# evandez/neuron-descriptions

Measured on AMD Instinct MI355X. Metric: neuron-descriptions/sec (whole node), 4096 neurons x k=15 exemplars, higher is better.
Workload: dtype f32-equivalent: operands split into (hi,lo) f16 pairs (22 significant bits), 3 f16 MFMAs per product, f32 accumulate

## Files before the change

### neuron-descriptions_amd/csrc/api.hip

```cpp
#include "common.h"

#include <cstdarg>
#include <cstdio>
#include <cstring>

namespace milan {

static thread_local char g_err[1024] = "";

void set_error(const char* fmt, ...) {
  va_list ap;
  va_start(ap, fmt);
  vsnprintf(g_err, sizeof(g_err), fmt, ap);
  va_end(ap);
}

int dev_alloc(milan_ctx* c, void** p, size_t bytes) {
  if (bytes == 0) bytes = 16;
  MILAN_CHECK_HIP(hipMalloc(p, (bytes + 255) & ~size_t(255)));
  c->owned.push_back(*p);
  return 0;
}

__global__ void absmax_kernel(const float* __restrict__ w, long n,
// ... 371 lines not shown
  MILAN_REQUIRE(c && seqs && out, MILAN_ERR_ARG,
                "milan_lm_logprobs: null argument");
  set_status_word(c->status);
  Arena a;
  MILAN_TRY(make_arena(workspace, workspace_bytes, &a));
  return decoder_lm_logprobs(c, seqs, rows, L, out, a, (hipStream_t)stream);
}

int milan_conv2d_nhwc(const float* x, int n, int h, int w, int cin,
                      const float* weight_oihw, const float* bias, int cout,
                      int kh, int kw, int stride, int pad, int relu,
                      const float* residual, float* y, int precision,
                      milan_stream stream) {
  MILAN_REQUIRE(x && weight_oihw && y, MILAN_ERR_ARG, "conv2d: null argument");
  set_status_word(nullptr);
  const bool force_strip = precision == 3, tap_major = precision == 4;
  if (force_strip || tap_major) precision = MILAN_PRECISION_SPLIT_F16;
  MILAN_REQUIRE(!force_strip || MILAN_EXPERIMENTS, MILAN_ERR_ARG,
                "conv2d: the LDS-strip 3x3 kernel is only in an experiments build "
                "(make EXPERIMENTS=1)");
  MILAN_REQUIRE(precision == MILAN_PRECISION_F32 || cin % 32 == 0,
                MILAN_ERR_SHAPE, "conv2d: split-f16 needs cin %% 32 == 0");
  MILAN_REQUIRE(cin % 4 == 0 && n > 0 && cout > 0, MILAN_ERR_SHAPE,
                "conv2d: cin must be a multiple of 4");
  hipStream_t s = (hipStream_t)stream;
  const int K = kh * kw * cin, Kp = (K + 31) / 32 * 32;
  float *wp = nullptr, *zero = nullptr, *xs = nullptr, *wsp = nullptr, *ws3 = nullptr, *wst = nullptr;
  MILAN_CHECK_HIP(hipMalloc((void**)&wp, sizeof(float) * (size_t)cout * Kp));
  MILAN_CHECK_HIP(hipMalloc((void**)&zero, 256));
  MILAN_CHECK_HIP(hipMemsetAsync(zero, 0, 256, s));
  int r = pack_conv_plain(weight_oihw, cout, cin, kh, kw, wp, s);
  if (r == 0) {
// ... 11 lines not shown
      hipError_t e1 = hipMalloc((void**)&xs, sizeof(float) * (size_t)rows * cin);
      hipError_t e2 = hipMalloc((void**)&wsp, sizeof(float) * (size_t)cout * Kp);
      if (e1 != hipSuccess || e2 != hipSuccess) {
        set_error("conv2d: out of memory");
        r = (int)hipErrorOutOfMemory;
      } else {
        r = launch_f32_to_split(x, cin, xs, cin, rows, cin, 1.f, s);
        if (r == 0)
          r = split_weight_into(wp, cout, Kp, wsp, &g.acc_scale,
                                reinterpret_cast<unsigned int*>(zero) + 32, s);
        g.A = xs; g.W = wsp; g.a_split = 1;
        if (r == 0 && !tap_major && kh * kw > 1 && kh * kw <= 32 && K == Kp) {
          if (hipMalloc((void**)&wst, sizeof(float) * (size_t)cout * Kp) == hipSuccess) {
            r = make_slice_major(wsp, cout, kh * kw, cin, 4, 2, wst, s);
            g.Wt = wst;
          }
        }
        if (MILAN_EXPERIMENTS && r == 0 && kh == 3 && kw == 3 && stride == 1 &&
            pad == 1 && K == Kp) {
          if (hipMalloc((void**)&ws3, sizeof(float) * (size_t)cout * Kp) == hipSuccess) {
            r = make_chunk_major(wsp, cout, cin, ws3, s);
            g.W3 = ws3;
            if (force_strip) g.tile_hint = 8;
          }
        }
      }
    }
    if (r == 0) r = launch_gemm(g, s);
  }
  hipError_t e = hipStreamSynchronize(s);
// ... 163 lines not shown
```

### neuron-descriptions_amd/csrc/common.h

```cpp
#pragma once
#include <hip/hip_runtime.h>
#include <stdint.h>
#include <stddef.h>
#include <string>
#include <vector>
#include <map>

#include "../../include/milan_hip.h"

#ifndef MILAN_EXPERIMENTS
#define MILAN_EXPERIMENTS 0
#endif

namespace milan {

void set_error(const char* fmt, ...);
#define MILAN_CHECK_HIP(expr)                                              \
  do {                                                                     \
    hipError_t _e = (expr);                                                \
    if (_e != hipSuccess) {                                                \
      milan::set_error("%s:%d: %s -> %s", __FILE__, __LINE__, #expr,       \
                       hipGetErrorString(_e));                             \
      return (int)_e;                                                      \
    }                                                                      \
// ... 10 lines not shown
    int _r = (expr);                                                       \
    if (_r != 0) return _r;                                                \
  } while (0)

enum Epilogue : int {
  EPI_BIAS = 0,
  EPI_BIAS_RELU = 1,
  EPI_BIAS_RES_RELU = 2,
  EPI_BIAS_TANH = 3,
  EPI_BIAS_SIGMUL = 4,
  EPI_BIAS_ADD = 5,
  EPI_LSTM = 6,
  EPI_LSE = 7,
};

struct GemmArgs {
  const float* A;
  const float* W;
  const float* bias;
  const float* aux;
  float* C;
  int M, N, K, Kp;
  int ldc, ldaux;
  int H, Wd, Cin, Ho, Wo, KH, KW, stride, pad;
  long a_pix_stride;
  long a_img_stride;
  int epilogue;
  const float* zero;
  int flop_k;
  int a_split;
// ... 10 lines not shown
  int tile_hint;
  int stagger;
  long long* prof;
  int chunk_major;
  float* C2;
  float* Cs;
  unsigned* status;
  int f16;
  const float* Wt;
  int tap_inner;
  const long long* lse_tgt;
  long lse_tgt_stride;
  float* lse_x;
  const int* m_live;
  int m_live_mul;
};

enum OutMode : int { OUT_SCALAR = 0, OUT_VEC4 = 1, OUT_SPLIT8 = 2, OUT_F16 = 3 };

int launch_gemm(const GemmArgs& g, hipStream_t s);
void set_status_word(unsigned* word);
unsigned* status_word();
void profile_tag_kernel(int family);
int launch_zero_fill(void* p, size_t bytes, hipStream_t s);
int launch_f32_to_split(const float* src, long ld_src, float* dst, long ld_dst,
                        long rows, int K, float scale, hipStream_t s);
int gemm_profile_enable(int enable);
int ensure_lds_attr(const void* kern, int bytes);
int device_cus8(int* out);
void* gemm_profile_begin(double flops, double bytes, hipStream_t s);
void gemm_profile_end(void* rec, hipStream_t s);
// ... 350 lines not shown
```

### neuron-descriptions_amd/csrc/gemm.hip

```cpp
#include "common.h"

#include <map>
#include <mutex>
#include <utility>

#include <cstdio>
#include <cstdlib>
#include <type_traits>
#include <utility>
#include <vector>

#ifndef MILAN_ABLATE_BUILD
#define MILAN_ABLATE_BUILD 0
#endif
#ifndef MILAN_EXPERIMENTS
#define MILAN_EXPERIMENTS 0
#endif

namespace milan {

typedef float f32x16 __attribute__((ext_vector_type(16)));
typedef float f32x4 __attribute__((ext_vector_type(4)));
typedef _Float16 f16x8 __attribute__((ext_vector_type(8)));

// ... 47 lines not shown
               "s_nop 1\n\tv_max_f32_dpp %0, %0, %0 quad_perm:[2,3,0,1] row_mask:0xf bank_mask:0xf\n\t"
               "s_nop 1\n\tv_max_f32_dpp %0, %0, %0 row_half_mirror row_mask:0xf bank_mask:0xf\n\t"
               "s_nop 1\n\tv_max_f32_dpp %0, %0, %0 row_mirror row_mask:0xf bank_mask:0xf"
               : "+v"(x));
  return x;
}
__device__ __forceinline__ float row16_sum(float x) {
  asm volatile("s_nop 1\n\tv_add_f32_dpp %0, %0, %0 quad_perm:[1,0,3,2] row_mask:0xf bank_mask:0xf\n\t"
               "s_nop 1\n\tv_add_f32_dpp %0, %0, %0 quad_perm:[2,3,0,1] row_mask:0xf bank_mask:0xf\n\t"
               "s_nop 1\n\tv_add_f32_dpp %0, %0, %0 row_half_mirror row_mask:0xf bank_mask:0xf\n\t"
               "s_nop 1\n\tv_add_f32_dpp %0, %0, %0 row_mirror row_mask:0xf bank_mask:0xf"
               : "+v"(x));
  return x;
}

template <int TM, int TN, bool SWZ64 = false>
__device__ __forceinline__ void run_epilogue(const GemmArgs& g,
                                             f32x16 (&acc)[TM][TN], float* smem,
                                             int wave, int lane, int row0,
                                             int col0) {
  static_assert(TN == 2, "epilogues assume 64-column wave tiles");
  constexpr int SROW = SWZ64 ? 64 : 68;
  auto sw = [](int row, int col) { return SWZ64 ? (col ^ ((row & 1) << 2)) : col; };
  float* stage_out = smem + wave * (32 * SROW);
  auto to_stage = [&](int i) {
#pragma unroll
    for (int j = 0; j < TN; ++j)
#pragma unroll
      for (int r = 0; r < 16; ++r) {
        const int row = (r & 3) + 8 * (r >> 2) + 4 * (lane >> 5);
        stage_out[row * SROW + sw(row, j * 32 + (lane & 31))] = acc[i][j][r];
      }
  };

  auto epilogue_vec4 = [&](auto epi_tag) {
    constexpr int EPI = decltype(epi_tag)::value;
    const int col4 = (lane & 15) * 4;
    const int n = col0 + col4;
    const bool n_ok = n < g.N;
    f32x4 bias4 = {0.f, 0.f, 0.f, 0.f};
    if (g.bias && n_ok) bias4 = *reinterpret_cast<const f32x4*>(g.bias + n);
    constexpr bool AUX = (EPI == EPI_BIAS_RES_RELU || EPI == EPI_BIAS_ADD ||
                          EPI == EPI_BIAS_SIGMUL);
    f32x4 res[AUX ? 2 : 1][8];
    auto load_res = [&](int i, f32x4 (&r)[8]) {
#pragma unroll
      for (int it = 0; it < 8; ++it) {
        const int m = row0 + i * 32 + it * 4 + (lane >> 4);
        r[it] = (m < g.M && n_ok)
                    ? *reinterpret_cast<const f32x4*>(g.aux + (long)m * g.ldaux + n)
                    : f32x4{0.f, 0.f, 0.f, 0.f};
      }
    };
    if constexpr (AUX) load_res(0, res[0]);
#pragma unroll
    for (int i = 0; i < TM; ++i) {
      if constexpr (AUX) {
        if (i + 1 < TM) load_res(i + 1, res[(i + 1) & 1]);
      }
      to_stage(i);
#pragma unroll
      for (int it = 0; it < 8; ++it) {
        const int row = it * 4 + (lane >> 4);
        const int m = row0 + i * 32 + row;
        f32x4 v = *reinterpret_cast<const f32x4*>(stage_out + row * SROW + sw(row, col4));
        if (m < g.M && n_ok) {
          v += bias4;
          if constexpr (AUX) {
            const f32x4 a = res[i & 1][it];
            if constexpr (EPI == EPI_BIAS_SIGMUL) {
#pragma unroll
              for (int e = 0; e < 4; ++e)
                v[e] = (1.f / (1.f + expf(-v[e]))) * a[e];
            } else {
              v += a;
            }
          }
          if constexpr (EPI == EPI_BIAS_RELU || EPI == EPI_BIAS_RES_RELU) {
#pragma unroll
// ... 8 lines not shown
      }
    }
  };

  auto epilogue_lse = [&]() {
    const int col4 = (lane & 15) * 4;
    const int n = col0 + col4;
    const bool n_ok = n < g.N;
    f32x4 bias4 = {0.f, 0.f, 0.f, 0.f};
    if (g.bias && n_ok) bias4 = *reinterpret_cast<const f32x4*>(g.bias + n);
    const int cb = col0 >> 6;
    int tg[2][8];
    auto load_tgt = [&](int i, int (&t)[8]) {
#pragma unroll
      for (int it = 0; it < 8; ++it) {
        const int m = row0 + i * 32 + it * 4 + (lane >> 4);
        t[it] = m < g.M ? (int)g.lse_tgt[(long)m * g.lse_tgt_stride] : -1;
      }
    };
    load_tgt(0, tg[0]);
#pragma unroll
    for (int i = 0; i < TM; ++i) {
      if (i + 1 < TM) load_tgt(i + 1, tg[(i + 1) & 1]);
      to_stage(i);
#pragma unroll
      for (int it = 0; it < 8; ++it) {
        const int row = it * 4 + (lane >> 4);
        const int m = row0 + i * 32 + row;
        f32x4 v = *reinterpret_cast<const f32x4*>(stage_out + row * SROW + sw(row, col4));
        v += bias4;
        const bool ok = m < g.M && n_ok;
        float mx = ok ? fmaxf(fmaxf(v[0], v[1]), fmaxf(v[2], v[3])) : -INFINITY;
        mx = row16_max(mx);
        float e = ok ? (__expf(v[0] - mx) + __expf(v[1] - mx)) + (__expf(v[2] - mx) + __expf(v[3] - mx)) : 0.f;
        e = row16_sum(e);
        if (m < g.M && col0 < g.N) {
          if ((lane & 15) == 0) {
            float* d = g.C + (long)m * g.ldc + 2 * cb;
            d[0] = mx;
            d[1] = e;
          }
          const int tgt = tg[i & 1][it];
          if (n_ok && tgt >= n && tgt < n + 4) {
// ... 12 lines not shown
    const bool n_ok = n < g.N;
    float bias8[8] = {0.f, 0.f, 0.f, 0.f, 0.f, 0.f, 0.f, 0.f};
    if (g.bias && n_ok) {
      const f32x4 b0 = *reinterpret_cast<const f32x4*>(g.bias + n);
      const f32x4 b1 = *reinterpret_cast<const f32x4*>(g.bias + n + 4);
#pragma unroll
      for (int e = 0; e < 4; ++e) { bias8[e] = b0[e]; bias8[4 + e] = b1[e]; }
    }
    constexpr bool SIG = EPI == EPI_BIAS_SIGMUL;
    constexpr bool RES = (EPI == EPI_BIAS_RES_RELU || EPI == EPI_BIAS_ADD || SIG);
    float sat = 0.f;
    f32x4 res[RES ? 2 : 1][4][2];
    auto load_res = [&](int i, f32x4 (&r)[4][2]) {
#pragma unroll
      for (int it = 0; it < 4; ++it) {
        const int m = row0 + i * 32 + it * 8 + (lane >> 3);
        if (m < g.M && n_ok) {
          const float* ap = g.aux + (long)m * g.ldaux + n;
          r[it][0] = *reinterpret_cast<const f32x4*>(ap);
          r[it][1] = *reinterpret_cast<const f32x4*>(ap + 4);
        } else {
          r[it][0] = f32x4{0.f, 0.f, 0.f, 0.f};
          r[it][1] = r[it][0];
        }
      }
    };
    if constexpr (RES) load_res(0, res[0]);
#pragma unroll
    for (int i = 0; i < TM; ++i) {
      if constexpr (RES) {
        if (i + 1 < TM) load_res(i + 1, res[(i + 1) & 1]);
      }
      to_stage(i);
#pragma unroll
      for (int it = 0; it < 4; ++it) {
        const int row = it * 8 + (lane >> 3);
        const int m = row0 + i * 32 + row;
        const f32x4 v0 =
            *reinterpret_cast<const f32x4*>(stage_out + row * SROW + sw(row, col8));
        const f32x4 v1 =
            *reinterpret_cast<const f32x4*>(stage_out + row * SROW + sw(row, col8 + 4));
        if (m < g.M && n_ok) {
          float v[8];
#pragma unroll
          for (int e = 0; e < 4; ++e) {
            v[e] = v0[e] + bias8[e];
            v[4 + e] = v1[e] + bias8[4 + e];
          }
          if constexpr (SIG) {
            const f32x4 a0 = res[i & 1][it][0], a1 = res[i & 1][it][1];
#pragma unroll
            for (int e = 0; e < 4; ++e) {
// ... 27 lines not shown
    const int n = col0 + col8;
    const bool n_ok = n < g.N;
    float bias8[8] = {0.f, 0.f, 0.f, 0.f, 0.f, 0.f, 0.f, 0.f};
    if (g.bias && n_ok) {
      const f32x4 b0 = *reinterpret_cast<const f32x4*>(g.bias + n);
      const f32x4 b1 = *reinterpret_cast<const f32x4*>(g.bias + n + 4);
#pragma unroll
      for (int e = 0; e < 4; ++e) { bias8[e] = b0[e]; bias8[4 + e] = b1[e]; }
    }
    constexpr bool RES = EPI == EPI_BIAS_RES_RELU;
    float sat = 0.f;
    f32x4 res[RES ? 2 : 1][4];
    auto load_res = [&](int i, f32x4 (&r)[4]) {
#pragma unroll
      for (int it = 0; it < 4; ++it) {
        const int m = row0 + i * 32 + it * 8 + (lane >> 3);
        r[it] = (m < g.M && n_ok)
                    ? *reinterpret_cast<const f32x4*>(reinterpret_cast<const char*>(g.aux) +
                                                      ((long)m * g.ldaux * 4 + n * 2))
                    : f32x4{0.f, 0.f, 0.f, 0.f};
      }
    };
    if constexpr (RES) load_res(0, res[0]);
#pragma unroll
    for (int i = 0; i < TM; ++i) {
      if constexpr (RES) {
        if (i + 1 < TM) load_res(i + 1, res[(i + 1) & 1]);
      }
      to_stage(i);
#pragma unroll
      for (int it = 0; it < 4; ++it) {
        const int row = it * 8 + (lane >> 3);
        const int m = row0 + i * 32 + row;
        const f32x4 v0 = *reinterpret_cast<const f32x4*>(stage_out + row * SROW + sw(row, col8));
        const f32x4 v1 = *reinterpret_cast<const f32x4*>(stage_out + row * SROW + sw(row, col8 + 4));
        if (m < g.M && n_ok) {
          float v[8];
#pragma unroll
          for (int e = 0; e < 4; ++e) {
            v[e] = v0[e] + bias8[e];
            v[4 + e] = v1[e] + bias8[4 + e];
          }
          if constexpr (RES) {
            const f16x8v a = __builtin_bit_cast(f16x8v, res[i & 1][it]);
#pragma unroll
            for (int e = 0; e < 8; ++e) v[e] += (float)a[e];
          }
          float x[8];
// ... 17 lines not shown

  auto epilogue_lstm = [&]() {
    const int q4 = (lane & 3) * 4;
    const int u = (col0 >> 2) + q4;
    const bool n_ok = col0 < g.N;
    f32x4 bias4[4];
#pragma unroll
    for (int gate = 0; gate < 4; ++gate)
      bias4[gate] = (g.bias && n_ok)
                        ? *reinterpret_cast<const f32x4*>(g.bias + col0 + gate * 16 + q4)
                        : f32x4{0.f, 0.f, 0.f, 0.f};
    f32x4 cin[2][2];
    auto load_c = [&](int i, f32x4 (&c)[2]) {
#pragma unroll
      for (int it = 0; it < 2; ++it) {
        const int m = row0 + i * 32 + it * 16 + (lane >> 2);
        c[it] = (m < g.M && n_ok)
                    ? *reinterpret_cast<const f32x4*>(g.aux + (long)m * g.ldaux + u)
                    : f32x4{0.f, 0.f, 0.f, 0.f};
      }
    };
    load_c(0, cin[0]);
#pragma unroll
    for (int i = 0; i < TM; ++i) {
      if (i + 1 < TM) load_c(i + 1, cin[(i + 1) & 1]);
      to_stage(i);
#pragma unroll
      for (int it = 0; it < 2; ++it) {
        const int row = it * 16 + (lane >> 2);
        const int m = row0 + i * 32 + row;
        f32x4 p[4];
#pragma unroll
        for (int gate = 0; gate < 4; ++gate)
          p[gate] = *reinterpret_cast<const f32x4*>(stage_out + row * SROW +
                                                    sw(row, gate * 16 + q4)) + bias4[gate];
        if (m < g.M && n_ok) {
          f32x4 h4, c4;
#pragma unroll
          for (int e = 0; e < 4; ++e) {
            float hh, cc;
            lstm_cell(p[0][e], p[1][e], p[2][e], p[3][e], cin[i & 1][it][e], &hh, &cc);
            h4[e] = hh; c4[e] = cc;
          }
          *reinterpret_cast<f32x4*>(g.C + (long)m * g.ldc + u) = h4;
          *reinterpret_cast<f32x4*>(g.C2 + (long)m * g.ldc + u) = c4;
// ... 14 lines not shown
          }
        }
      }
    }
  };

  auto epilogue_scalar = [&](auto epi_tag) {
    constexpr int EPI = decltype(epi_tag)::value;
#pragma unroll
    for (int j = 0; j < TN; ++j) {
      const int n = col0 + j * 32 + (lane & 31);
      if (n >= g.N) continue;
      const float bias = g.bias ? g.bias[n] : 0.f;
#pragma unroll
      for (int i = 0; i < TM; ++i) {
        const int mbase = row0 + i * 32 + 4 * (lane >> 5);
#pragma unroll
        for (int r = 0; r < 16; ++r) {
          const int m = mbase + (r & 3) + 8 * (r >> 2);
          if (m >= g.M) continue;
          float v = acc[i][j][r] + bias;
          if constexpr (EPI == EPI_BIAS_RELU) v = fmaxf(v, 0.f);
          if constexpr (EPI == EPI_BIAS_RES_RELU)
            v = fmaxf(v + g.aux[(long)m * g.ldaux + n], 0.f);
          if constexpr (EPI == EPI_BIAS_ADD) v = v + g.aux[(long)m * g.ldaux + n];
          if constexpr (EPI == EPI_BIAS_TANH) v = tanhf(v);
          if constexpr (EPI == EPI_BIAS_SIGMUL)
            v = (1.f / (1.f + expf(-v))) * g.aux[(long)m * g.ldaux + n];
          g.C[(long)m * g.ldc + n] = v;
        }
      }
    }
  };

// ... 988 lines not shown
  __builtin_amdgcn_s_barrier();
  const GemmArgs ge = reload_gemm_args();
#pragma unroll
  for (int i = 0; i < TM; ++i)
#pragma unroll
    for (int j = 0; j < TN; ++j) acc[i][j] = acc[i][j] * ge.acc_scale;
  run_epilogue<TM, TN>(ge, acc, smem, wave, lane, tile_m * BM + wm * 128, tile_n * BN + wn * 64);
}

struct PpLoader {
  __amdgpu_buffer_rsrc_t srd_a, srd_a2, srd_w, cur_srd;
  unsigned row_off[4], row_off2[4], voff[4], vb[4];
  int hw0[4];
  unsigned mask[4];
  int ia, iw, is_kh, is_kw, is_cin0, seg_soff, cin_limit;
};

template <int BNW, bool F16 = false, bool TAPI = false>
__device__ __forceinline__ void split16_pp32_tile(int tile_m, int tile_n, int tid, bool prefetched,
                                                  bool has_next, int ntile_m, int ntile_n) {
  const GemmArgs g = reload_gemm_args();
  constexpr int BM = 256, BN = 256, BKP = 32, TM = BNW == 256 ? 4 : 2, TN = 2;
  static_assert(BNW == 256 || BNW == 128, "ping-pong tile: 256 or 128 columns");
  constexpr int SLOTF = BM * BKP;
  constexpr unsigned OOB = 0x80000000u;
  extern __shared__ __attribute__((aligned(16))) float smem[];
  auto a_slot = [&](int sl) { return smem + (sl < 2 ? sl : 3) * SLOTF; };
  auto w_slot = [&](int sl) { return smem + (sl == 0 ? 2 : 4) * SLOTF; };
  const int lane = tid & 63;
  const int wave = __builtin_amdgcn_readfirstlane(tid >> 6);
  const int wm = BNW == 256 ? wave >> 2 : wave >> 1, wn = BNW == 256 ? wave & 3 : wave & 1;
  const int group = wave >> 2;
  const int HoWo = g.Ho * g.Wo;
  const int np = g.Kp / BKP;
  const int k1_pairs = g.A2 ? g.K1 / BKP : 0x7fffffff;

  auto set_tap = [&](PpLoader& L) {
    if constexpr (TAPI) {
      const int t = L.is_kh * g.KW + L.is_kw;
#pragma unroll
      for (int it = 0; it < 4; ++it) L.voff[it] = (L.mask[it] >> t) & 1u ? L.row_off[it] : OOB;
      L.seg_soff = (int)((((long)L.is_kh * g.Wd + L.is_kw) * g.a_pix_stride) * 4);
      return;
    }
#pragma unroll
    for (int it = 0; it < 4; ++it) {
      const int hi = (L.hw0[it] >> 16) + L.is_kh, wi = (int)(short)(L.hw0[it] & 0xffff) + L.is_kw;
      const bool inb = (unsigned)hi < (unsigned)g.H && (unsigned)wi < (unsigned)g.Wd;
      L.voff[it] = inb ? L.row_off[it] : OOB;
    }
    L.seg_soff = (int)((((long)L.is_kh * g.Wd + L.is_kw) * g.a_pix_stride) * 4);
  };
  auto setup = [&](PpLoader& L, int tm, int tn) {
    const int prow = lane >> 3, pos = lane & 7;
    const int m0 = tm * BM;
    const int img0 = m0 / HoWo;
    const int rem0 = m0 - img0 * HoWo;
    const long bias = ((long)g.pad * g.Wd + g.pad) * g.a_pix_stride;
    L.srd_a = __builtin_amdgcn_make_buffer_rsrc(
        const_cast<float*>(g.A + (long)img0 * g.a_img_stride - bias), 0, 0x7fffffff, 0x00020000);
    L.srd_a2 = __builtin_amdgcn_make_buffer_rsrc(
        const_cast<float*>(g.A2 ? g.A2 + (long)img0 * g.a2_img_stride : g.A), 0, 0x7fffffff,
        0x00020000);
    L.srd_w = __builtin_amdgcn_make_buffer_rsrc(const_cast<float*>(g.W + (long)tn * BNW * g.Kp), 0,
                                                0x7fffffff, 0x00020000);
    const float r_howo = 1.0f / (float)HoWo, r_wo = 1.0f / (float)g.Wo;
#pragma unroll
    for (int it = 0; it < 4; ++it) {
      const int row = it * 64 + wave * 8 + prow;
      const int q = pos ^ ((row >> 1) & 7);
      const bool ok = m0 + row < g.M;
      const int x = rem0 + (ok ? row : 0);
      int dimg = (int)((float)x * r_howo);
      dimg -= (dimg * HoWo > x);
      dimg += ((dimg + 1) * HoWo <= x);
      const int rem = x - dimg * HoWo;
      int ho = (int)((float)rem * r_wo);
      ho -= (ho * g.Wo > rem);
      ho += ((ho + 1) * g.Wo <= rem);
      const int wo = rem - ho * g.Wo;
      const int hi0 = ho * g.stride - g.pad, wi0 = wo * g.stride - g.pad;
      L.hw0[it] = (hi0 << 16) | (wi0 & 0xffff);
      if constexpr (TAPI) {
        unsigned m = 0;
        for (int kh = 0, t = 0; kh < g.KH; ++kh)
          for (int kw = 0; kw < g.KW; ++kw, ++t)
            m |= (unsigned)((unsigned)(hi0 + kh) < (unsigned)g.H &&
                            (unsigned)(wi0 + kw) < (unsigned)g.Wd) << t;
        L.mask[it] = m;
      }
      L.row_off[it] = ok ? (unsigned)(((long)dimg * g.a_img_stride +
                                       ((long)hi0 * g.Wd + wi0) * g.a_pix_stride + bias + q * 4) * 4)
                         : OOB;
      L.row_off2[it] = (ok && g.A2)
                           ? (unsigned)(((long)dimg * g.a2_img_stride +
                                         ((long)(ho * g.stride2) * g.W2d + wo * g.stride2) *
                                             g.a2_pix_stride + q * 4) * 4)
                           : OOB;
      L.vb[it] = (row < BNW && tn * BNW + row < g.N) ? (unsigned)(((long)row * g.Kp + q * 4) * 4) : OOB;
    }
    L.ia = L.iw = L.is_kh = L.is_kw = L.is_cin0 = 0;
    L.cin_limit = g.Cin;
    L.cur_srd = L.srd_a;
    set_tap(L);
  };
  auto issue_a = [&](PpLoader& L, auto slot_tag, bool really) {
    constexpr int SLOT = decltype(slot_tag)::value;
    if (really) {
      int woff = wave * (8 * BKP);
      asm volatile("" : "+s"(woff));
      float* dst = a_slot(SLOT) + woff;
      const int soff = L.seg_soff + L.is_cin0 * 4;
#pragma unroll
      for (int it = 0; it < 4; ++it)
        __builtin_amdgcn_raw_ptr_buffer_load_lds(L.cur_srd, (LDS_AS void*)(dst + it * (64 * BKP)), 16,
                                                 L.voff[it], soff, 0, 0);
    }
    if constexpr (TAPI) {
      if (L.ia + 1 < np) {
        ++L.ia;
        if (++L.is_kw == g.KW) {
          L.is_kw = 0;
          if (++L.is_kh == g.KH) { L.is_kh = 0; L.is_cin0 += BKP; }
        }
        set_tap(L);
      }
      return;
    }
    if (L.ia + 1 < np) {
      ++L.ia;
      L.is_cin0 += BKP;
      if (L.ia == k1_pairs) {
        L.cur_srd = L.srd_a2;
#pragma unroll
        for (int it = 0; it < 4; ++it) L.voff[it] = L.row_off2[it];
        L.seg_soff = 0;
        L.is_cin0 = 0;
        L.cin_limit = 0x7fffffff;
      } else if (L.is_cin0 >= L.cin_limit) {
        L.is_cin0 = 0;
        if (++L.is_kw == g.KW) { L.is_kw = 0; ++L.is_kh; }
        set_tap(L);
      }
    }
  };
  auto issue_w = [&](PpLoader& L, auto slot_tag, bool really) {
    constexpr int SLOT = decltype(slot_tag)::value;
    if (really) {
      int woff = wave * (8 * BKP);
      asm volatile("" : "+s"(woff));
      float* dst = w_slot(SLOT) + woff;
      const int soff = L.iw * (BKP * 4);
#pragma unroll
      for (int it = 0; it < (BNW == 256 ? 4 : 2); ++it)
        __builtin_amdgcn_raw_ptr_buffer_load_lds(L.srd_w, (LDS_AS void*)(dst + it * (64 * BKP)), 16,
                                                 L.vb[it], soff, 0, 0);
    }
    if (L.iw + 1 < np) ++L.iw;
  };
  using I0 = std::integral_constant<int, 0>;
  using I1 = std::integral_constant<int, 1>;

  PpLoader L;
  setup(L, tile_m, tile_n);

  const int frow = lane & 31, fhalf = lane >> 5;
  const int fsw = (frow >> 1) & 7;
  const float* a_p[2][2];
  const float* a_q[2][2];
  const float* b_p[2][2];
  const float* b_q[2][2];
#pragma unroll
  for (int sl = 0; sl < 2; ++sl)
// ... 154 lines not shown
  }
  asm volatile("s_waitcnt vmcnt(0)" ::: "memory");
  __builtin_amdgcn_s_barrier();
  if (has_next) {
    PpLoader N;
    setup(N, ntile_m, ntile_n);
    issue_a(N, I0{}, true);
    issue_w(N, I0{}, true);
    issue_a(N, I1{}, true);
  }
  const GemmArgs ge = reload_gemm_args();
#pragma unroll
  for (int i = 0; i < TM; ++i)
#pragma unroll
    for (int j = 0; j < TN; ++j) acc[i][j] = acc[i][j] * ge.acc_scale;
  run_epilogue<TM, TN, true>(ge, acc, a_slot(2), wave, lane, tile_m * BM + wm * (TM * 32),
                             tile_n * BNW + wn * 64);
}

template <int BNW>
__global__ __launch_bounds__(512, 2) void igemm_split16_pp32n_kernel(GemmArgs g, int tiles_m,
                                                                     int tiles_n) {
  tiles_m = live_tiles_m(g, tiles_m, 256);
  const int T = tiles_m * tiles_n;
  int q = blockIdx.x;
  if (q >= T) return;
  bool prefetched = false;
  for (;;) {
    const int tile = xcd_tile(q, T);
    const int tile_m = tile / tiles_n, tile_n = tile - tile_m * tiles_n;
    const bool has_next = q + (int)gridDim.x < T;
    int ntile_m = tile_m, ntile_n = tile_n;
// ... 18 lines not shown
  tiles_m = live_tiles_m(g, tiles_m, 256);
  const int T = tiles_m * tiles_n;
  const int q = blockIdx.x;
  if (q >= T) return;
  const int tile = xcd_tile(q, T);
  const int tile_m = tile / tiles_n, tile_n = tile - tile_m * tiles_n;
  int tid = threadIdx.x;
  asm volatile("" : "+v"(tid));
  split16_pp32_tile<256>(tile_m, tile_n, tid, false, false, tile_m, tile_n);
}

template <int BNW>
__global__ __launch_bounds__(512, 2) void igemm_split16_pp32t_kernel(GemmArgs g, int tiles_m,
                                                                     int tiles_n) {
  tiles_m = live_tiles_m(g, tiles_m, 256);
  const int T = tiles_m * tiles_n;
  const int q = blockIdx.x;
  if (q >= T) return;
  const int tile = xcd_tile(q, T);
  const int tile_m = tile / tiles_n, tile_n = tile - tile_m * tiles_n;
  int tid = threadIdx.x;
  asm volatile("" : "+v"(tid));
  split16_pp32_tile<BNW, false, true>(tile_m, tile_n, tid, false, false, tile_m, tile_n);
}

template <int BNW, bool TAPI>
__global__ __launch_bounds__(512, 2) void igemm_f16_pp32_kernel(GemmArgs g, int tiles_m, int tiles_n) {
  tiles_m = live_tiles_m(g, tiles_m, 256);
  const int T = tiles_m * tiles_n;
  const int q = blockIdx.x;
  if (q >= T) return;
  const int tile = xcd_tile(q, T);
  const int tile_m = tile / tiles_n, tile_n = tile - tile_m * tiles_n;
  int tid = threadIdx.x;
  asm volatile("" : "+v"(tid));
  split16_pp32_tile<BNW, true, TAPI>(tile_m, tile_n, tid, false, false, tile_m, tile_n);
}

__global__ __launch_bounds__(512, 2) void igemm_split16_pp_kernel(GemmArgs g, int tiles_m,
                                                                  int tiles_n) {
  tiles_m = live_tiles_m(g, tiles_m, 256);
  const int T = tiles_m * tiles_n;
  for (int q = blockIdx.x; q < T; q += gridDim.x) {
    const int tile = xcd_tile(q, T);
    const int tile_m = tile / tiles_n;
    int tid = threadIdx.x;
    asm volatile("" : "+v"(tid));
    split16_pp_tile(tile_m, tile - tile_m * tiles_n, tid);
    __builtin_amdgcn_s_barrier();
  }
}
// ... 465 lines not shown
  auto kern = igemm_split16_tm2_kernel<BM, BN, STAGES>;
  MILAN_TRY(ensure_lds_attr(reinterpret_cast<const void*>(kern), (int)lds));
  hipLaunchKernelGGL(kern, dim3(tiles_m * tiles_n), dim3(NT), lds, s, g, tiles_m,
                     tiles_n);
  MILAN_CHECK_HIP(hipGetLastError());
  return 0;
}

static bool tap_inner_wanted(const GemmArgs& g) {
  static int on = -1;
  if (on < 0) { const char* e = getenv("MILAN_TAP_INNER"); on = e ? atoi(e) : 1; }
  return on && g.Wt && !g.A2 && g.KH * g.KW > 1 && g.KH * g.KW <= 32 && g.K == g.Kp &&
         g.Cin % 32 == 0;
}

template <int BNW>
static int launch_split16_pp32(const GemmArgs& g, hipStream_t s) {
  const int tiles_m = (g.M + 255) / 256, tiles_n = (g.N + BNW - 1) / BNW;
  const size_t lds = size_t(5) * 256 * 32 * sizeof(float);
  if (tap_inner_wanted(g)) {
    GemmArgs t = g;
    t.W = g.Wt;
    t.tap_inner = 1;
    profile_tag_kernel(BNW == 256 ? MILAN_KERNEL_PP32T_256 : MILAN_KERNEL_PP32_128);
    auto kern = igemm_split16_pp32t_kernel<BNW>;
    MILAN_TRY(ensure_lds_attr(reinterpret_cast<const void*>(kern), (int)lds));
    hipLaunchKernelGGL(kern, dim3(tiles_m * tiles_n), dim3(512), lds, s, t, tiles_m, tiles_n);
    MILAN_CHECK_HIP(hipGetLastError());
    return 0;
  }
  int ncus = 0;
  MILAN_TRY(device_cus8(&ncus));
  int grid = tiles_m * tiles_n;
  static int persist = -1;
  if (persist < 0) { const char* e = getenv("MILAN_PP_PERSIST"); persist = e ? atoi(e) : 0; }
  const bool walk = persist && (persist != 2 || g.K <= 512) && grid > ncus;
  profile_tag_kernel(BNW == 256 ? MILAN_KERNEL_PP32_256 : MILAN_KERNEL_PP32_128);
  if (BNW == 256 && !walk) {
    auto kern = igemm_split16_pp32_kernel;
    MILAN_TRY(ensure_lds_attr(reinterpret_cast<const void*>(kern), (int)lds));
    hipLaunchKernelGGL(kern, dim3(grid), dim3(512), lds, s, g, tiles_m, tiles_n);
  } else {
// ... 3 lines not shown
    hipLaunchKernelGGL(kern, dim3(grid), dim3(512), lds, s, g, tiles_m, tiles_n);
  }
  MILAN_CHECK_HIP(hipGetLastError());
  return 0;
}

template <int BNW>
static int launch_f16_pp32(const GemmArgs& g, hipStream_t s) {
  const int tiles_m = (g.M + 255) / 256, tiles_n = (g.N + BNW - 1) / BNW;
  const size_t lds = size_t(5) * 256 * 32 * sizeof(float);
  profile_tag_kernel(MILAN_KERNEL_F16);
  if (tap_inner_wanted(g)) {
    GemmArgs t = g;
    t.W = g.Wt;
    t.tap_inner = 1;
    auto kern = igemm_f16_pp32_kernel<BNW, true>;
    MILAN_TRY(ensure_lds_attr(reinterpret_cast<const void*>(kern), (int)lds));
    hipLaunchKernelGGL(kern, dim3(tiles_m * tiles_n), dim3(512), lds, s, t, tiles_m, tiles_n);
    MILAN_CHECK_HIP(hipGetLastError());
    return 0;
  }
  auto kern = igemm_f16_pp32_kernel<BNW, false>;
  MILAN_TRY(ensure_lds_attr(reinterpret_cast<const void*>(kern), (int)lds));
  hipLaunchKernelGGL(kern, dim3(tiles_m * tiles_n), dim3(512), lds, s, g, tiles_m, tiles_n);
  MILAN_CHECK_HIP(hipGetLastError());
  return 0;
}

static int launch_split16_pp(const GemmArgs& g, hipStream_t s) {
  const int tiles_m = (g.M + 255) / 256, tiles_n = (g.N + 255) / 256;
  const size_t lds = size_t(4) * (256 + 256) * 16 * sizeof(float);
  static_assert(size_t(4) * 512 * 16 * sizeof(float) >= size_t(8) * 32 * 68 * sizeof(float),
                "the epilogue stages through the ring");
// ... 273 lines not shown
```

### neuron-descriptions_amd/milan_amd/hip.py

```python
import ctypes
import os
import pathlib
import weakref
from typing import Dict, Optional, Sequence, Tuple

import torch

LIB_PATH = pathlib.Path(os.environ.get('MILAN_LIB') or
                       pathlib.Path(__file__).resolve().parent / 'lib' / 'libmilan_hip.so')
EXP_LIB_PATH = pathlib.Path(__file__).resolve().parent / 'lib' / 'libmilan_hip_exp.so'

GREEDY, FORCED, BEAM, RERANK = 0, 1, 2, 3
PRECISION_F32, PRECISION_SPLIT_F16, PRECISION_F16 = 0, 1, 2
PRECISIONS = {'f32': PRECISION_F32, 'split_f16': PRECISION_SPLIT_F16, 'f16': PRECISION_F16}
FUSE_CHAIN, FUSE_CHAIN_WIDE, FUSE_STEM, FUSE_CONV3, FUSE_SKIP_EMPTY, FUSE_BNECK, FUSE_SPARSE_TAIL = 1, 2, 4, 8, 16, 32, 64
SKETCH_COMPACT, SKETCH_INSERT, SKETCH_MOVE, SKETCH_HALVE = 0, 1, 2, 3
STATUS_SATURATED, STATUS_NONFINITE_INPUT = 1, 2
KERNEL_FAMILIES = ('other', 'pp32_256', 'pp32_128', 'split_other', 'f32', 'chain',
                   'chain_wide', 'stem', 'conv3', 'f16', 'pp32t_256', 'bneck')


class SketchOp(ctypes.Structure):
    _fields_ = [('kind', ctypes.c_int32), ('src', ctypes.c_int32),
                ('dst', ctypes.c_int32), ('offset', ctypes.c_int32),
                ('extremes', ctypes.c_int32), ('reserved', ctypes.c_int32),
                ('n', ctypes.c_int64), ('position', ctypes.c_int64),
                ('capacity', ctypes.c_int64)]


DRAW_BIT = ctypes.CFUNCTYPE(ctypes.c_int, ctypes.c_void_p)
_CONV_PRECISIONS = dict(f32=0, split_f16=1, split_f16_strip=3, split_f16_tap_major=4)
DTYPE_U8, DTYPE_F32 = 0, 1

ERR_ARG, ERR_SHAPE, ERR_STATE, ERR_WORKSPACE, ERR_NO_LM = -1, -2, -3, -4, -5


class HipUnavailableError(RuntimeError):
    """libmilan_hip.so or a HIP device is missing."""


class Dims(ctypes.Structure):
    _fields_ = [
        ('trunk_width', ctypes.c_int32),
        ('trunk_blocks', ctypes.c_int32 * 4),
        ('feature_size', ctypes.c_int32),
        ('hidden_size', ctypes.c_int32),
# ... 1451 lines not shown
```

Measured before the change: 1313.

## Skip padded taps in tap-inner conv GEMM by grouping output pixels into border classes

Output pixels of the tap-inner implicit-GEMM conv are partitioned into up to nine classes by which kernel taps fall inside the image (interior vs. border rows/columns). Each class gets its own block range and iterates only over its valid taps via a bitmask, so the zero-padding taps at borders are no longer loaded or multiplied. The epilogue now scatters rows through a per-wave LDS row table because a tile no longer covers contiguous output rows. This adds grid bookkeeping, an env toggle, and an extra tile-rounding loss per class, in exchange for skipping the wasted padding work.

```diff
diff --git a/neuron-descriptions_amd/csrc/api.hip b/neuron-descriptions_amd/csrc/api.hip
--- a/neuron-descriptions_amd/csrc/api.hip
+++ b/neuron-descriptions_amd/csrc/api.hip
@@ -409,8 +409,8 @@
                       milan_stream stream) {
   MILAN_REQUIRE(x && weight_oihw && y, MILAN_ERR_ARG, "conv2d: null argument");
   set_status_word(nullptr);
-  const bool force_strip = precision == 3, tap_major = precision == 4;
-  if (force_strip || tap_major) precision = MILAN_PRECISION_SPLIT_F16;
+  const bool force_strip = precision == 3, tap_major = precision == 4, tap_linear = precision == 5;
+  if (force_strip || tap_major || tap_linear) precision = MILAN_PRECISION_SPLIT_F16;
   MILAN_REQUIRE(!force_strip || MILAN_EXPERIMENTS, MILAN_ERR_ARG,
                 "conv2d: the LDS-strip 3x3 kernel is only in an experiments build "
                 "(make EXPERIMENTS=1)");
@@ -452,6 +452,7 @@
           if (hipMalloc((void**)&wst, sizeof(float) * (size_t)cout * Kp) == hipSuccess) {
             r = make_slice_major(wsp, cout, kh * kw, cin, 4, 2, wst, s);
             g.Wt = wst;
+            if (tap_linear) g.tap_ncls = -1;
           }
         }
         if (MILAN_EXPERIMENTS && r == 0 && kh == 3 && kw == 3 && stride == 1 &&
diff --git a/neuron-descriptions_amd/csrc/common.h b/neuron-descriptions_amd/csrc/common.h
--- a/neuron-descriptions_amd/csrc/common.h
+++ b/neuron-descriptions_amd/csrc/common.h
@@ -48,6 +48,7 @@
   EPI_LSE = 7,
 };
 
+constexpr int MILAN_TAP_CLASSES = 9;
 struct GemmArgs {
   const float* A;
   const float* W;
@@ -88,7 +89,10 @@
   float* lse_x;
   const int* m_live;
   int m_live_mul;
-};
+  int tap_ncls;
+  int tap_cls[MILAN_TAP_CLASSES][5];
+};
+static_assert(sizeof(GemmArgs) % 4 == 0, "GemmArgs is reloaded word by word");
 
 enum OutMode : int { OUT_SCALAR = 0, OUT_VEC4 = 1, OUT_SPLIT8 = 2, OUT_F16 = 3 };
 
diff --git a/neuron-descriptions_amd/csrc/gemm.hip b/neuron-descriptions_amd/csrc/gemm.hip
--- a/neuron-descriptions_amd/csrc/gemm.hip
+++ b/neuron-descriptions_amd/csrc/gemm.hip
@@ -6,6 +6,7 @@
 
 #include <cstdio>
 #include <cstdlib>
+#include <cstring>
 #include <type_traits>
 #include <utility>
 #include <vector>
@@ -85,12 +86,16 @@
   return x;
 }
 
-template <int TM, int TN, bool SWZ64 = false>
+template <int TM, int TN, bool SWZ64 = false, bool ROWTAB = false>
 __device__ __forceinline__ void run_epilogue(const GemmArgs& g,
                                              f32x16 (&acc)[TM][TN], float* smem,
                                              int wave, int lane, int row0,
-                                             int col0) {
+                                             int col0, const int* rowtab = nullptr) {
   static_assert(TN == 2, "epilogues assume 64-column wave tiles");
+  auto out_row = [&](int r) {
+    if constexpr (ROWTAB) return rowtab[r];
+    else return row0 + r;
+  };
   constexpr int SROW = SWZ64 ? 64 : 68;
   auto sw = [](int row, int col) { return SWZ64 ? (col ^ ((row & 1) << 2)) : col; };
   float* stage_out = smem + wave * (32 * SROW);
@@ -117,7 +122,7 @@
     auto load_res = [&](int i, f32x4 (&r)[8]) {
 #pragma unroll
       for (int it = 0; it < 8; ++it) {
-        const int m = row0 + i * 32 + it * 4 + (lane >> 4);
+        const int m = out_row(i * 32 + it * 4 + (lane >> 4));
         r[it] = (m < g.M && n_ok)
                     ? *reinterpret_cast<const f32x4*>(g.aux + (long)m * g.ldaux + n)
                     : f32x4{0.f, 0.f, 0.f, 0.f};
@@ -133,7 +138,7 @@
 #pragma unroll
       for (int it = 0; it < 8; ++it) {
         const int row = it * 4 + (lane >> 4);
-        const int m = row0 + i * 32 + row;
+        const int m = out_row(i * 32 + row);
         f32x4 v = *reinterpret_cast<const f32x4*>(stage_out + row * SROW + sw(row, col4));
         if (m < g.M && n_ok) {
           v += bias4;
@@ -172,7 +177,7 @@
     auto load_tgt = [&](int i, int (&t)[8]) {
 #pragma unroll
       for (int it = 0; it < 8; ++it) {
-        const int m = row0 + i * 32 + it * 4 + (lane >> 4);
+        const int m = out_row(i * 32 + it * 4 + (lane >> 4));
         t[it] = m < g.M ? (int)g.lse_tgt[(long)m * g.lse_tgt_stride] : -1;
       }
     };
@@ -184,7 +189,7 @@
 #pragma unroll
       for (int it = 0; it < 8; ++it) {
         const int row = it * 4 + (lane >> 4);
-        const int m = row0 + i * 32 + row;
+        const int m = out_row(i * 32 + row);
         f32x4 v = *reinterpret_cast<const f32x4*>(stage_out + row * SROW + sw(row, col4));
         v += bias4;
         const bool ok = m < g.M && n_ok;
@@ -227,7 +232,7 @@
     auto load_res = [&](int i, f32x4 (&r)[4][2]) {
 #pragma unroll
       for (int it = 0; it < 4; ++it) {
-        const int m = row0 + i * 32 + it * 8 + (lane >> 3);
+        const int m = out_row(i * 32 + it * 8 + (lane >> 3));
         if (m < g.M && n_ok) {
           const float* ap = g.aux + (long)m * g.ldaux + n;
           r[it][0] = *reinterpret_cast<const f32x4*>(ap);
@@ -248,7 +253,7 @@
 #pragma unroll
       for (int it = 0; it < 4; ++it) {
         const int row = it * 8 + (lane >> 3);
-        const int m = row0 + i * 32 + row;
+        const int m = out_row(i * 32 + row);
         const f32x4 v0 =
             *reinterpret_cast<const f32x4*>(stage_out + row * SROW + sw(row, col8));
         const f32x4 v1 =
@@ -306,7 +311,7 @@
     auto load_res = [&](int i, f32x4 (&r)[4]) {
 #pragma unroll
       for (int it = 0; it < 4; ++it) {
-        const int m = row0 + i * 32 + it * 8 + (lane >> 3);
+        const int m = out_row(i * 32 + it * 8 + (lane >> 3));
         r[it] = (m < g.M && n_ok)
                     ? *reinterpret_cast<const f32x4*>(reinterpret_cast<const char*>(g.aux) +
                                                       ((long)m * g.ldaux * 4 + n * 2))
@@ -323,7 +328,7 @@
 #pragma unroll
       for (int it = 0; it < 4; ++it) {
         const int row = it * 8 + (lane >> 3);
-        const int m = row0 + i * 32 + row;
+        const int m = out_row(i * 32 + row);
         const f32x4 v0 = *reinterpret_cast<const f32x4*>(stage_out + row * SROW + sw(row, col8));
         const f32x4 v1 = *reinterpret_cast<const f32x4*>(stage_out + row * SROW + sw(row, col8 + 4));
         if (m < g.M && n_ok) {
@@ -371,7 +376,7 @@
     auto load_c = [&](int i, f32x4 (&c)[2]) {
 #pragma unroll
       for (int it = 0; it < 2; ++it) {
-        const int m = row0 + i * 32 + it * 16 + (lane >> 2);
+        const int m = out_row(i * 32 + it * 16 + (lane >> 2));
         c[it] = (m < g.M && n_ok)
                     ? *reinterpret_cast<const f32x4*>(g.aux + (long)m * g.ldaux + u)
                     : f32x4{0.f, 0.f, 0.f, 0.f};
@@ -385,7 +390,7 @@
 #pragma unroll
       for (int it = 0; it < 2; ++it) {
         const int row = it * 16 + (lane >> 2);
-        const int m = row0 + i * 32 + row;
+        const int m = out_row(i * 32 + row);
         f32x4 p[4];
 #pragma unroll
         for (int gate = 0; gate < 4; ++gate)
@@ -430,10 +435,9 @@
       const float bias = g.bias ? g.bias[n] : 0.f;
 #pragma unroll
       for (int i = 0; i < TM; ++i) {
-        const int mbase = row0 + i * 32 + 4 * (lane >> 5);
 #pragma unroll
         for (int r = 0; r < 16; ++r) {
-          const int m = mbase + (r & 3) + 8 * (r >> 2);
+          const int m = out_row(i * 32 + 4 * (lane >> 5) + (r & 3) + 8 * (r >> 2));
           if (m >= g.M) continue;
           float v = acc[i][j][r] + bias;
           if constexpr (EPI == EPI_BIAS_RELU) v = fmaxf(v, 0.f);
@@ -1452,11 +1456,56 @@
   int hw0[4];
   unsigned mask[4];
   int ia, iw, is_kh, is_kw, is_cin0, seg_soff, cin_limit;
+  unsigned a_bits, w_bits;
+  int w_slice;
 };
+
+struct TapTile {
+  int y0, ny, x0, nx;
+  unsigned mask;
+  int cnt, j, tile_n;
+};
+
+__device__ __forceinline__ bool tap_tile(const GemmArgs& g, int tiles_m, int tiles_n, TapTile* t) {
+  const int b = blockIdx.x;
+  if (g.tap_ncls == 0) {
+    const int T = tiles_m * tiles_n;
+    if (b >= T) return false;
+    const int tile = xcd_tile(b, T);
+    t->j = tile / tiles_n;
+    t->tile_n = tile - t->j * tiles_n;
+    t->y0 = 0; t->ny = g.Ho; t->x0 = 0; t->nx = g.Wo;
+    t->mask = 0xffffffffu >> (32 - g.KH * g.KW);
+    t->cnt = g.M;
+    return true;
+  }
+  typedef const int __attribute__((address_space(4)))* KArgWords;
+  const KArgWords cw = (KArgWords)__builtin_amdgcn_kernarg_segment_ptr() + offsetof(GemmArgs, tap_cls) / 4;
+  const int imgs = g.M / (g.Ho * g.Wo);
+  int first = 0, cls = -1, cfirst = 0, ctiles = 0;
+#pragma unroll
+  for (int c = 0; c < MILAN_TAP_CLASSES; ++c) {
+    const int T = c < g.tap_ncls ? ((imgs * cw[c * 5 + 1] * cw[c * 5 + 3] + 255) >> 8) * tiles_n : 0;
+    const int B = (T + 7) & ~7;
+    if (cls < 0 && b < first + B) { cls = c; cfirst = first; ctiles = T; }
+    first += B;
+  }
+  if (cls < 0) return false;
+  const int bl = b - cfirst;
+  if ((bl >> 3) >= (ctiles >> 3) + ((bl & 7) < (ctiles & 7))) return false;
+  const int tile = xcd_tile(bl, ctiles);
+  t->j = tile / tiles_n;
+  t->tile_n = tile - t->j * tiles_n;
+  t->y0 = cw[cls * 5]; t->ny = cw[cls * 5 + 1]; t->x0 = cw[cls * 5 + 2]; t->nx = cw[cls * 5 + 3];
+  t->mask = (unsigned)cw[cls * 5 + 4];
+  t->cnt = imgs * t->ny * t->nx;
+  return true;
+}
 
 template <int BNW, bool F16 = false, bool TAPI = false>
 __device__ __forceinline__ void split16_pp32_tile(int tile_m, int tile_n, int tid, bool prefetched,
-                                                  bool has_next, int ntile_m, int ntile_n) {
+                                                  bool has_next, int ntile_m, int ntile_n,
+                                                  TapTile tt = TapTile{}) {
   const GemmArgs g = reload_gemm_args();
   constexpr int BM = 256, BN = 256, BKP = 32, TM = BNW == 256 ? 4 : 2, TN = 2;
   static_assert(BNW == 256 || BNW == 128, "ping-pong tile: 256 or 128 columns");
@@ -1470,15 +1519,18 @@
   const int wm = BNW == 256 ? wave >> 2 : wave >> 1, wn = BNW == 256 ? wave & 3 : wave & 1;
   const int group = wave >> 2;
   const int HoWo = g.Ho * g.Wo;
-  const int np = g.Kp / BKP;
+  const int np = TAPI ? (g.Cin / BKP) * __builtin_popcount(tt.mask) : g.Kp / BKP;
   const int k1_pairs = g.A2 ? g.K1 / BKP : 0x7fffffff;
+  const int KHKW = g.KH * g.KW;
+  const int r_kw = 65536 / g.KW + 1;
 
   auto set_tap = [&](PpLoader& L) {
     if constexpr (TAPI) {
-      const int t = L.is_kh * g.KW + L.is_kw;
+      const int t = __builtin_ctz(L.a_bits);
+      const int kh = (t * r_kw) >> 16, kw = t - kh * g.KW;
 #pragma unroll
       for (int it = 0; it < 4; ++it) L.voff[it] = (L.mask[it] >> t) & 1u ? L.row_off[it] : OOB;
-      L.seg_soff = (int)((((long)L.is_kh * g.Wd + L.is_kw) * g.a_pix_stride) * 4);
+      L.seg_soff = (int)((((long)kh * g.Wd + kw) * g.a_pix_stride) * 4);
       return;
     }
 #pragma unroll
@@ -1489,11 +1541,29 @@
     }
     L.seg_soff = (int)((((long)L.is_kh * g.Wd + L.is_kw) * g.a_pix_stride) * 4);
   };
+  const int pix_img = TAPI ? tt.ny * tt.nx : HoWo, pix_row = TAPI ? tt.nx : g.Wo;
+  const int rows_all = TAPI ? tt.cnt : g.M;
+  const float r_howo = 1.0f / (float)pix_img, r_wo = 1.0f / (float)pix_row;
+  auto row_pixel = [&](int m0, int rem0, int row, int* dimg_out, int* ho_out, int* wo_out) {
+    const bool ok = m0 + row < rows_all;
+    const int x = rem0 + (ok ? row : 0);
+    int dimg = (int)((float)x * r_howo);
+    dimg -= (dimg * pix_img > x);
+    dimg += ((dimg + 1) * pix_img <= x);
+    const int rem = x - dimg * pix_img;
+    int ho = (int)((float)rem * r_wo);
+    ho -= (ho * pix_row > rem);
+    ho += ((ho + 1) * pix_row <= rem);
+    *dimg_out = dimg;
+    *wo_out = rem - ho * pix_row + (TAPI ? tt.x0 : 0);
+    *ho_out = ho + (TAPI ? tt.y0 : 0);
+    return ok;
+  };
   auto setup = [&](PpLoader& L, int tm, int tn) {
     const int prow = lane >> 3, pos = lane & 7;
     const int m0 = tm * BM;
-    const int img0 = m0 / HoWo;
-    const int rem0 = m0 - img0 * HoWo;
+    const int img0 = m0 / pix_img;
+    const int rem0 = m0 - img0 * pix_img;
     const long bias = ((long)g.pad * g.Wd + g.pad) * g.a_pix_stride;
     L.srd_a = __builtin_amdgcn_make_buffer_rsrc(
         const_cast<float*>(g.A + (long)img0 * g.a_img_stride - bias), 0, 0x7fffffff, 0x00020000);
@@ -1502,21 +1572,12 @@
         0x00020000);
     L.srd_w = __builtin_amdgcn_make_buffer_rsrc(const_cast<float*>(g.W + (long)tn * BNW * g.Kp), 0,
                                                 0x7fffffff, 0x00020000);
-    const float r_howo = 1.0f / (float)HoWo, r_wo = 1.0f / (float)g.Wo;
 #pragma unroll
     for (int it = 0; it < 4; ++it) {
       const int row = it * 64 + wave * 8 + prow;
       const int q = pos ^ ((row >> 1) & 7);
-      const bool ok = m0 + row < g.M;
-      const int x = rem0 + (ok ? row : 0);
-      int dimg = (int)((float)x * r_howo);
-      dimg -= (dimg * HoWo > x);
-      dimg += ((dimg + 1) * HoWo <= x);
-      const int rem = x - dimg * HoWo;
-      int ho = (int)((float)rem * r_wo);
-      ho -= (ho * g.Wo > rem);
-      ho += ((ho + 1) * g.Wo <= rem);
-      const int wo = rem - ho * g.Wo;
+      int dimg, ho, wo;
+      const bool ok = row_pixel(m0, rem0, row, &dimg, &ho, &wo);
       const int hi0 = ho * g.stride - g.pad, wi0 = wo * g.stride - g.pad;
       L.hw0[it] = (hi0 << 16) | (wi0 & 0xffff);
       if constexpr (TAPI) {
@@ -1538,6 +1599,8 @@
       L.vb[it] = (row < BNW && tn * BNW + row < g.N) ? (unsigned)(((long)row * g.Kp + q * 4) * 4) : OOB;
     }
     L.ia = L.iw = L.is_kh = L.is_kw = L.is_cin0 = 0;
+    L.a_bits = L.w_bits = tt.mask;
+    L.w_slice = 0;
     L.cin_limit = g.Cin;
     L.cur_srd = L.srd_a;
     set_tap(L);
@@ -1557,10 +1620,8 @@
     if constexpr (TAPI) {
       if (L.ia + 1 < np) {
         ++L.ia;
-        if (++L.is_kw == g.KW) {
-          L.is_kw = 0;
-          if (++L.is_kh == g.KH) { L.is_kh = 0; L.is_cin0 += BKP; }
-        }
+        L.a_bits &= L.a_bits - 1;
+        if (L.a_bits == 0) { L.a_bits = tt.mask; L.is_cin0 += BKP; }
         set_tap(L);
       }
       return;
@@ -1588,13 +1649,19 @@
       int woff = wave * (8 * BKP);
       asm volatile("" : "+s"(woff));
       float* dst = w_slot(SLOT) + woff;
-      const int soff = L.iw * (BKP * 4);
+      const int soff = (TAPI ? L.w_slice * KHKW + (int)__builtin_ctz(L.w_bits) : L.iw) * (BKP * 4);
 #pragma unroll
       for (int it = 0; it < (BNW == 256 ? 4 : 2); ++it)
         __builtin_amdgcn_raw_ptr_buffer_load_lds(L.srd_w, (LDS_AS void*)(dst + it * (64 * BKP)), 16,
                                                  L.vb[it], soff, 0, 0);
     }
-    if (L.iw + 1 < np) ++L.iw;
+    if (L.iw + 1 < np) {
+      ++L.iw;
+      if constexpr (TAPI) {
+        L.w_bits &= L.w_bits - 1;
+        if (L.w_bits == 0) { L.w_bits = tt.mask; ++L.w_slice; }
+      }
+    }
   };
   using I0 = std::integral_constant<int, 0>;
   using I1 = std::integral_constant<int, 1>;
@@ -1779,8 +1846,23 @@
   for (int i = 0; i < TM; ++i)
 #pragma unroll
     for (int j = 0; j < TN; ++j) acc[i][j] = acc[i][j] * ge.acc_scale;
-  run_epilogue<TM, TN, true>(ge, acc, a_slot(2), wave, lane, tile_m * BM + wm * (TM * 32),
-                             tile_n * BNW + wn * 64);
+  if constexpr (TAPI) {
+    int* tab = reinterpret_cast<int*>(a_slot(0)) + wave * (TM * 32);
+    const int m0 = tile_m * BM;
+    const int img0 = m0 / pix_img;
+    const int rem0 = m0 - img0 * pix_img;
+#pragma unroll
+    for (int e = 0; e < TM * 32 / 64; ++e) {
+      const int r = e * 64 + lane;
+      int dimg, ho, wo;
+      const bool ok = row_pixel(m0, rem0, wm * (TM * 32) + r, &dimg, &ho, &wo);
+      tab[r] = ok ? ((img0 + dimg) * ge.Ho + ho) * ge.Wo + wo : 0x7fffffff;
+    }
+    run_epilogue<TM, TN, true, true>(ge, acc, a_slot(2), wave, lane, 0, tile_n * BNW + wn * 64, tab);
+  } else {
+    run_epilogue<TM, TN, true>(ge, acc, a_slot(2), wave, lane, tile_m * BM + wm * (TM * 32),
+                               tile_n * BNW + wn * 64);
+  }
 }
 
 template <int BNW>
@@ -1829,27 +1911,32 @@
 __global__ __launch_bounds__(512, 2) void igemm_split16_pp32t_kernel(GemmArgs g, int tiles_m,
                                                                      int tiles_n) {
   tiles_m = live_tiles_m(g, tiles_m, 256);
-  const int T = tiles_m * tiles_n;
-  const int q = blockIdx.x;
-  if (q >= T) return;
-  const int tile = xcd_tile(q, T);
-  const int tile_m = tile / tiles_n, tile_n = tile - tile_m * tiles_n;
+  TapTile tt;
+  if (!tap_tile(g, tiles_m, tiles_n, &tt)) return;
   int tid = threadIdx.x;
   asm volatile("" : "+v"(tid));
-  split16_pp32_tile<BNW, false, true>(tile_m, tile_n, tid, false, false, tile_m, tile_n);
+  split16_pp32_tile<BNW, false, true>(tt.j, tt.tile_n, tid, false, false, tt.j, tt.tile_n, tt);
 }
 
 template <int BNW, bool TAPI>
 __global__ __launch_bounds__(512, 2) void igemm_f16_pp32_kernel(GemmArgs g, int tiles_m, int tiles_n) {
   tiles_m = live_tiles_m(g, tiles_m, 256);
-  const int T = tiles_m * tiles_n;
-  const int q = blockIdx.x;
-  if (q >= T) return;
-  const int tile = xcd_tile(q, T);
-  const int tile_m = tile / tiles_n, tile_n = tile - tile_m * tiles_n;
-  int tid = threadIdx.x;
-  asm volatile("" : "+v"(tid));
-  split16_pp32_tile<BNW, true, TAPI>(tile_m, tile_n, tid, false, false, tile_m, tile_n);
+  if constexpr (TAPI) {
+    TapTile tt;
+    if (!tap_tile(g, tiles_m, tiles_n, &tt)) return;
+    int tid = threadIdx.x;
+    asm volatile("" : "+v"(tid));
+    split16_pp32_tile<BNW, true, true>(tt.j, tt.tile_n, tid, false, false, tt.j, tt.tile_n, tt);
+  } else {
+    const int T = tiles_m * tiles_n;
+    const int q = blockIdx.x;
+    if (q >= T) return;
+    const int tile = xcd_tile(q, T);
+    const int tile_m = tile / tiles_n, tile_n = tile - tile_m * tiles_n;
+    int tid = threadIdx.x;
+    asm volatile("" : "+v"(tid));
+    split16_pp32_tile<BNW, true, false>(tile_m, tile_n, tid, false, false, tile_m, tile_n);
+  }
 }
 
 __global__ __launch_bounds__(512, 2) void igemm_split16_pp_kernel(GemmArgs g, int tiles_m,
@@ -2345,6 +2432,59 @@
          g.Cin % 32 == 0;
 }
 
+static int tap_classes(GemmArgs& t, int tiles_m, int tiles_n) {
+  static int on = -1;
+  if (on < 0) { const char* e = getenv("MILAN_TAP_SKIP"); on = e ? atoi(e) : 1; }
+  const bool wanted = on && t.tap_ncls >= 0;
+  t.tap_ncls = 0;
+  const int howo = t.Ho * t.Wo;
+  if (!wanted || howo <= 0 || t.M % howo != 0 || (t.m_live && t.m_live_mul % howo != 0))
+    return tiles_m * tiles_n;
+  struct Run { int o0, n; unsigned set; };
+  auto runs = [](int size, int out, int k, int stride, int pad, Run* r) {
+    int n = 0;
+    for (int o = 0; o < out; ++o) {
+      unsigned set = 0;
+      for (int i = 0; i < k; ++i)
+        if (o * stride - pad + i >= 0 && o * stride - pad + i < size) set |= 1u << i;
+      if (n > 0 && r[n - 1].set == set) { ++r[n - 1].n; continue; }
+      if (n == MILAN_TAP_CLASSES) return MILAN_TAP_CLASSES + 1;
+      r[n++] = Run{o, 1, set};
+    }
+    return n;
+  };
+  Run ry[MILAN_TAP_CLASSES], rx[MILAN_TAP_CLASSES];
+  const int nry = runs(t.H, t.Ho, t.KH, t.stride, t.pad, ry);
+  const int nrx = runs(t.Wd, t.Wo, t.KW, t.stride, t.pad, rx);
+  if (nry * nrx > MILAN_TAP_CLASSES) return tiles_m * tiles_n;
+  int cls[MILAN_TAP_CLASSES][5], n = 0, min_pix = howo;
+  for (int a = 0; a < nry; ++a)
+    for (int b = 0; b < nrx; ++b, ++n) {
+      unsigned mask = 0;
+      for (int kh = 0; kh < t.KH; ++kh)
+        for (int kw = 0; kw < t.KW; ++kw)
+          if ((ry[a].set >> kh & 1u) && (rx[b].set >> kw & 1u)) mask |= 1u << (kh * t.KW + kw);
+      if (mask == 0) return tiles_m * tiles_n;
+      const int c[5] = {ry[a].o0, ry[a].n, rx[b].o0, rx[b].n, (int)mask};
+      int at = n;
+      while (at > 0 && __builtin_popcount((unsigned)cls[at - 1][4]) < __builtin_popcount(mask)) {
+        memcpy(cls[at], cls[at - 1], sizeof(c));
+        --at;
+      }
+      memcpy(cls[at], c, sizeof(c));
+      if (ry[a].n * rx[b].n < min_pix) min_pix = ry[a].n * rx[b].n;
+    }
+  if ((256L / min_pix + 2) * t.a_img_stride * 4 + 64 >= 0x7fffffffL) return tiles_m * tiles_n;
+  const long imgs = t.M / howo;
+  long grid = 0;
+  for (int c = 0; c < n; ++c)
+    grid += ((imgs * cls[c][1] * cls[c][3] + 255) / 256 * tiles_n + 7) / 8 * 8;
+  if (grid >= 0x7fffffffL) return tiles_m * tiles_n;
+  t.tap_ncls = n;
+  memcpy(t.tap_cls, cls, sizeof(int) * 5 * n);
+  return (int)grid;
+}
+
 template <int BNW>
 static int launch_split16_pp32(const GemmArgs& g, hipStream_t s) {
   const int tiles_m = (g.M + 255) / 256, tiles_n = (g.N + BNW - 1) / BNW;
@@ -2353,10 +2493,11 @@
     GemmArgs t = g;
     t.W = g.Wt;
     t.tap_inner = 1;
+    const int grid = tap_classes(t, tiles_m, tiles_n);
     profile_tag_kernel(BNW == 256 ? MILAN_KERNEL_PP32T_256 : MILAN_KERNEL_PP32_128);
     auto kern = igemm_split16_pp32t_kernel<BNW>;
     MILAN_TRY(ensure_lds_attr(reinterpret_cast<const void*>(kern), (int)lds));
-    hipLaunchKernelGGL(kern, dim3(tiles_m * tiles_n), dim3(512), lds, s, t, tiles_m, tiles_n);
+    hipLaunchKernelGGL(kern, dim3(grid), dim3(512), lds, s, t, tiles_m, tiles_n);
     MILAN_CHECK_HIP(hipGetLastError());
     return 0;
   }
@@ -2390,9 +2531,10 @@
     GemmArgs t = g;
     t.W = g.Wt;
     t.tap_inner = 1;
+    const int grid = tap_classes(t, tiles_m, tiles_n);
     auto kern = igemm_f16_pp32_kernel<BNW, true>;
     MILAN_TRY(ensure_lds_attr(reinterpret_cast<const void*>(kern), (int)lds));
-    hipLaunchKernelGGL(kern, dim3(tiles_m * tiles_n), dim3(512), lds, s, t, tiles_m, tiles_n);
+    hipLaunchKernelGGL(kern, dim3(grid), dim3(512), lds, s, t, tiles_m, tiles_n);
     MILAN_CHECK_HIP(hipGetLastError());
     return 0;
   }
diff --git a/neuron-descriptions_amd/milan_amd/hip.py b/neuron-descriptions_amd/milan_amd/hip.py
--- a/neuron-descriptions_amd/milan_amd/hip.py
+++ b/neuron-descriptions_amd/milan_amd/hip.py
@@ -29,7 +29,8 @@
 
 
 DRAW_BIT = ctypes.CFUNCTYPE(ctypes.c_int, ctypes.c_void_p)
-_CONV_PRECISIONS = dict(f32=0, split_f16=1, split_f16_strip=3, split_f16_tap_major=4)
+_CONV_PRECISIONS = dict(f32=0, split_f16=1, split_f16_strip=3, split_f16_tap_major=4,
+                        split_f16_tap_linear=5)
 DTYPE_U8, DTYPE_F32 = 0, 1
 
 ERR_ARG, ERR_SHAPE, ERR_STATE, ERR_WORKSPACE, ERR_NO_LM = -1, -2, -3, -4, -5
```

After: 1331, median of 6. 1.4% higher.
